# RaptorMai/online-continual-learning

Measured on NVIDIA H100. Metric: replay-step images/sec (ASER+SCR, ResNet18, CIFAR100), higher is better.
Workload: dtype f32

## Files before the change

include/b200ocl.h:

```cpp
#ifndef B200OCL_H_
#define B200OCL_H_

#include <stddef.h>
#include <stdint.h>

#ifdef __cplusplus
extern "C" {
#endif

#define B200OCL_OK 0
#define B200OCL_EINVAL 1
#define B200OCL_EUNSUPPORTED 2
#define B200OCL_EWORKSPACE 3
#define B200OCL_ECUDA 4

#define B200OCL_KNN_MAX_CAND 1024
#define B200OCL_KNN_MAX_CAND_LARGE 262144

const char* b200ocl_last_error(void);
int b200ocl_version(void);
uint64_t b200ocl_launch_count(void);
void b200ocl_profile_begin(void);
int b200ocl_profile_end(void);
int b200ocl_profile_get(int k, char* name, int name_len, double* ms, int* launches, double* work);
// ... 57 lines not shown
#define B200OCL_NET_MAX_DIM 4096

typedef struct {
  int in_h, in_w;
  int nf;
  int num_classes;
  int head;
  int feat_dim;
} b200ocl_net_desc;

typedef struct {
  float* params;
  float* grads;
  float* packed;
  float* bn_stats;
  int64_t* bn_tracked;
} b200ocl_net_state;

typedef struct {
  size_t n_params, n_packed, n_bn_stats;
  int n_bn, n_tensors, dim_in, out_dim;
} b200ocl_net_info;
int b200ocl_net_query(const b200ocl_net_desc* desc, b200ocl_net_info* info);
int b200ocl_net_tensor(const b200ocl_net_desc* desc, int i, size_t* offset, size_t* numel, int* has_grad);

int b200ocl_net_pack(const b200ocl_net_desc* desc, const b200ocl_net_state* st, void* stream);


size_t b200ocl_net_eval_workspace_bytes(const b200ocl_net_desc* desc, int N);
int b200ocl_net_features_eval(const b200ocl_net_desc* desc, const b200ocl_net_state* st, const float* x, int N,
                              float* feat, void* workspace, size_t workspace_bytes, void* stream);

size_t b200ocl_net_train_workspace_bytes(const b200ocl_net_desc* desc, int N);

typedef struct {
  size_t bytes;
  size_t z, a, mean, invstd;
  size_t feat, hid, proj;
  size_t wg_part, wg_layer;
  int cin, cout, ks, stride, hout, wout;
  int bn_fused, bn_grid;
  int wgrad_kernel, wgrad_splits;
  int sms;
} b200ocl_net_ws_layout;
int b200ocl_net_train_ws_layout(const b200ocl_net_desc* desc, int N, int layer, b200ocl_net_ws_layout* out);

typedef struct {
  int kernel;
  int nt, bn, pt, kwarps;
  int grid_x, grid_y;
  int th, tw, ti;
  size_t stat_bytes, stat_region;
  int sms;
} b200ocl_conv_geom;
int b200ocl_net_conv_geom(const b200ocl_net_desc* desc, int N, int layer, int pass, int sms, b200ocl_conv_geom* out);

int b200ocl_net_forward_train(const b200ocl_net_desc* desc, const b200ocl_net_state* st, const float* x, int N,
                              float* out, void* workspace, size_t workspace_bytes, void* stream);

int b200ocl_net_forward_evalgrad(const b200ocl_net_desc* desc, const b200ocl_net_state* st, const float* x, int N,
                                 float* out, void* workspace, size_t workspace_bytes, void* stream);

int b200ocl_net_forward_train_deferred(const b200ocl_net_desc* desc, const b200ocl_net_state* st, const float* x, int N,
                                       float* out, void* workspace, size_t workspace_bytes, void* stream);
int b200ocl_net_apply_running_stats(const b200ocl_net_desc* desc, const b200ocl_net_state* st, int N, void* workspace,
                                    size_t workspace_bytes, void* stream);

int b200ocl_net_backward(const b200ocl_net_desc* desc, const b200ocl_net_state* st, const float* x, const float* dout,
                         int N, void* workspace, size_t workspace_bytes, int accumulate, void* stream);

int b200ocl_net_sgd_step(const b200ocl_net_desc* desc, const b200ocl_net_state* st, float lr, float weight_decay,
                         const b200ocl_net_state* dst, void* stream);

size_t b200ocl_net_sgd_step_clipped_workspace_bytes(const b200ocl_net_desc* desc);
int b200ocl_net_sgd_step_clipped(const b200ocl_net_desc* desc, const b200ocl_net_state* st, float lr,
                                 float weight_decay, float max_norm, float* norm_out, void* workspace,
                                 size_t workspace_bytes, void* stream);

typedef struct {
  float* running;
  float* tmp;
  float* normalized;
  float* prev;
} b200ocl_ewc_state;

#define B200OCL_EWC_PENALTY 1
#define B200OCL_EWC_EMA 2

size_t b200ocl_net_sgd_step_ewc_workspace_bytes(const b200ocl_net_desc* desc);
int b200ocl_net_sgd_step_ewc(const b200ocl_net_desc* desc, const b200ocl_net_state* st, const b200ocl_ewc_state* ewc,
                             float lr, float weight_decay, float up, int flags, float ema_keep, float ema_add,
                             float* penalty_out, void* workspace, size_t workspace_bytes, void* stream);

typedef struct {
  float step_size, bc2_sqrt, bc2_sqrt_inv, eps, beta1_c, beta2, beta2_c, weight_decay, grad_scale;
} b200ocl_adam_scalars;

#define B200OCL_ADAM_FOREACH 1
#define B200OCL_ADAM_GRAD_SCALE 2

int b200ocl_adam_step(float* p, float* g, float* m, float* v, size_t n, const b200ocl_adam_scalars* s, int flags,
                      void* stream);

typedef struct {
  float* exp_avg;
  float* exp_avg_sq;
// ... 53 lines not shown
```

online-continual-learning_b200/csrc/conv.cu:

```cuda
#include "conv.cuh"

namespace b200ocl {
namespace {

constexpr int CONV_THREADS = 128;

__device__ __forceinline__ double warp_sum_d(double v) {
#pragma unroll
  for (int o = 16; o > 0; o >>= 1) v += __shfl_xor_sync(FULL_MASK, v, o);
  return v;
}

__device__ __forceinline__ void decode_pixel(const ConvArgs& a, int m, int& n, int& ho, int& wo) {
  if (a.parity_order) {
    const int hh = a.Hout >> 1, wh = a.Wout >> 1;
    const int mq = a.N * hh * wh;
    const int cls = m / mq;
    int idx = m - cls * mq;
    n = idx / (hh * wh);
    idx -= n * hh * wh;
    const int y = idx / wh;
    ho = 2 * y + (cls >> 1);
    wo = 2 * (idx - y * wh) + (cls & 1);
  } else {
// ... 634 lines not shown
  return B200OCL_OK;
}

int launch_stem(const ConvArgs& a, const ConvPlan& pl, cudaStream_t stream) {
  B200OCL_PROF(a.mode == CONV_EVAL ? "conv_eval" : "conv_train", 2.0 * a.M * 20.0 * 27.0, stream);
  stem_kernel<<<pl.grid_x, CONV_THREADS, 0, stream>>>(a);
  B200OCL_LAUNCHED();
  return B200OCL_OK;
}

ConvPlan none(const char* why) {
  ConvPlan pl{};
  pl.kernel = CONV_K_NONE;
  pl.why = why;
  return pl;
}

ConvPlan tiled(const ConvArgs& a, int kernel, int bn, int pt, int bm) {
  ConvPlan pl{};
  pl.kernel = kernel;
  pl.bn = bn;
  pl.pt = pt;
  pl.grid_x = (a.M + bm - 1) / bm;
  pl.grid_y = a.CN / bn;
  return pl;
}

}

ConvPlan conv_plan(const ConvArgs& a, int sms) {
  if (a.CK == 3) {
    if (a.CN != 20 || a.ks != 3 || a.stride != 1 || a.Hin != a.Hout || a.Win != a.Wout || a.M <= 0 || a.transposed)
      return none("only the 3->20 3x3 stride-1 stem is supported");
    return tiled(a, CONV_K_STEM, 20, 1, CONV_THREADS);
  }
  if (a.CK % 20 != 0 || a.CN % 20 != 0 || a.M <= 0) return none("channel counts must be multiples of 20");
  ConvPlan pl{};
  bool tcp = false, tc = false;
  if (a.force_path == 3) {
    if (!conv_tcp_eligible(a)) return none("launch not covered by the halo-patch tensor-core kernel (3x3 stride 1, no train mode)");
    tcp = true;
  } else if (a.force_path == 2) {
    if (!(a.w_tc && a.ks == 3 && a.stride == 1 && !a.transposed)) return none("shape not covered by conv_tc");
    tc = true;
  } else if (a.force_path == 0) {
    tcp = conv_tcp_eligible(a);
    tc = !tcp && conv_tc_eligible(a, sms);
  }
  if (tcp) {
    pl.kernel = CONV_K_TCP;
    pl.nt = a.tp_bn <= 20 ? 32 : 48;
    pl.grid_x = conv_tcp_grid_x(a, sms);
    pl.grid_y = a.CN / a.tp_bn;
    return pl;
  }
  if (tc) {
    pl.kernel = CONV_K_TC;
    pl.nt = a.tc_bn <= 20 ? 32 : (a.tc_bn <= 40 ? 48 : 80);
    pl.grid_x = (a.M + 127) / 128;
    pl.grid_y = a.CN / a.tc_bn;
    return pl;
  }
  if (!a.transposed && a.ks * a.ks * 20 * 80 * sizeof(float) <= 64 * 1024) {
    const long want3 = 5L * sms / 2;
    const int pbn[3] = {80, 40, 20};
    const int ppt[3] = {4, 2, 1};
    for (int pi = 0; pi < 3; ++pi)
      for (int bi = 0; bi < 3; ++bi) {
        if (a.CN % pbn[bi]) continue;
        const PatchTile t = patch_tile(a, pbn[bi], ppt[pi]);
        const long need = (ppt[pi] == 4) ? 3L * sms / 2 : want3;
        if (t.ctas < need || t.smem > (ppt[pi] == 4 ? 100 : 72) * 1024) continue;
        pl.kernel = CONV_K_PATCH;
        pl.bn = pbn[bi];
        pl.pt = ppt[pi];
        pl.grid_y = a.CN / pl.bn;
        pl.grid_x = (int)(t.ctas / pl.grid_y);
        pl.th = t.th; pl.tw = t.tw; pl.ti = t.ti;
        pl.smem = t.smem;
        return pl;
      }
  }
  const long want = 4L * sms;
  const int bns[3] = {80, 40, 20};
  auto ctas_reg = [&](int bn, int pt) {
    const int bm = (80 / bn) * 32 * pt;
    return (long)((a.M + bm - 1) / bm) * (a.CN / bn);
  };
  for (int bi = 0; bi < 3; ++bi)
    if (a.CN % bns[bi] == 0 && ctas_reg(bns[bi], 2) >= want) return tiled(a, CONV_K_TILED, bns[bi], 2, (80 / bns[bi]) * 64);
  if (a.ks * a.ks * (a.CK / 20) >= 4) {
    int pt = 1, kwarps = 4;
    const long ctas2 = (long)((a.M + 63) / 64) * (a.CN / 20);
    const long ctas1 = (long)((a.M + 31) / 32) * (a.CN / 20);
    if (ctas2 >= want) pt = 2;
    else if (ctas1 < 2L * sms && a.ks * a.ks * (a.CK / 20) >= 16) kwarps = 8;
    pl = tiled(a, CONV_K_KSPLIT, 20, pt, 32 * pt);
    pl.kwarps = kwarps;
    return pl;
  }
  return tiled(a, CONV_K_TILED, 20, 1, 128);
}

int launch_conv(const ConvArgs& a, int sms, cudaStream_t stream) {
  const ConvPlan pl = conv_plan(a, sms);
  switch (pl.kernel) {
// ... 33 lines not shown
```

online-continual-learning_b200/csrc/conv.cuh:

```cuda
#pragma once
#include "common.cuh"

namespace b200ocl {

enum ConvMode {
  CONV_RAW = 0,
  CONV_EVAL = 1,
  CONV_TRAIN = 2,
  CONV_ACCUM = 3
};

struct ConvArgs {
  const float* in;
  const float* w;
  float* out;
  int N, Hin, Win, CK, Hout, Wout, CN;
  int ks, stride, pad;
  int transposed;
  const float* w_tc;
  int tc_kb, tc_bn;
  const float* w_tp;
  int tp_bn, tp_slices;
  int tp_ps, tp_bs, tp_tiles;
  int force_path;
// ... 4 lines not shown
  int mode;
  const float* gamma;
  const float* beta;
  const float* rmean;
  const float* rvar;
  const float* residual;
  int relu;
  float eps;
  double* stat_part;
  unsigned int* counter;
  float* save_mean;
  float* save_invstd;
  float* run_mean;
  float* run_var;
  float momentum;
};

__device__ __forceinline__ float bn_running_update(float run, float s, float m) {
  return __fmaf_rn(1.f - m, run, __fmul_rn(m, s));
}

__device__ __forceinline__ void bn_finalize(const ConvArgs& a, int c, double S, double Q) {
  const double cnt = (double)a.M;
  const double mean = S / cnt;
  double var = Q / cnt - mean * mean;
  if (var < 0.0) var = 0.0;
  a.save_mean[c] = (float)mean;
  a.save_invstd[c] = (float)(1.0 / sqrt(var + (double)a.eps));
  const double unbiased = (a.M > 1) ? var * cnt / (cnt - 1.0) : var;
  a.run_mean[c] = bn_running_update(a.run_mean[c], (float)mean, a.momentum);
  a.run_var[c] = bn_running_update(a.run_var[c], (float)unbiased, a.momentum);
}

constexpr int TP_LD_MAX = 13;
inline bool tcp_strip_fits(int W) { return 128 + 2 * (W + 2) + 2 <= 16 * TP_LD_MAX; }

enum ConvKernel {
  CONV_K_NONE = -1,
  CONV_K_STEM = 0,
  CONV_K_TCP = 1,
  CONV_K_TC = 2,
  CONV_K_PATCH = 3,
  CONV_K_TILED = 4,
  CONV_K_KSPLIT = 5
};
struct ConvPlan {
  int kernel;
  int nt;
  int bn, pt;
  int kwarps;
  int grid_x, grid_y;
  int th, tw, ti;
  size_t smem;
  const char* why;
};
ConvPlan conv_plan(const ConvArgs& a, int sms);
inline size_t conv_stat_bytes(const ConvPlan& pl, int CN) { return (size_t)pl.grid_x * CN * 2 * sizeof(double); }
int launch_conv(const ConvArgs& a, int sms, cudaStream_t stream);
bool conv_tc_eligible(const ConvArgs& a, int sms);
int launch_conv_tc(const ConvArgs& a, const ConvPlan& pl, cudaStream_t stream);
bool conv_tcp_eligible(const ConvArgs& a);
int conv_tcp_grid_x(const ConvArgs& a, int sms);
int launch_conv_tcp(const ConvArgs& a, const ConvPlan& pl, cudaStream_t stream);

}
```

online-continual-learning_b200/csrc/conv_tcp.cu:

```cuda
#include "conv.cuh"
#include "umma.cuh"

namespace b200ocl {
namespace {

constexpr int TP_THREADS = 32 * 13;
constexpr int TP_LOADER_WARP = 9;
constexpr int TP_PS_MAX = 3;
constexpr int TP_BS_MAX = 6;
constexpr int TP_CONSUMER_WARPS = 8;

using umma::mbar_expect_tx;
using umma::bulk_g2s;

struct TileGeom {
  int wp, pp;
  int tiles_m;
  int prow;
  int pbytes;
};
__host__ __device__ inline TileGeom tile_geom(int N, int H, int W) {
  TileGeom g;
  g.wp = W + 1;
  g.pp = (H + 1) * (W + 1);
  const long last = (long)(N - 1) * g.pp + (long)(H - 1) * g.wp + (W - 1);
  g.tiles_m = (int)(last / 128) + 1;
  g.prow = 128 + 2 * g.wp + 2;
  g.pbytes = (g.prow * 128 + 1023) / 1024 * 1024;
  return g;
}

template <int NT, int KS>
__device__ __forceinline__ void issue_tap(float (&d)[NT / 2], uint64_t dAh, uint64_t dAl, uint64_t dBh, uint64_t dBl) {
  umma::fence();
#pragma unroll
  for (int k = 0; k < KS; ++k) {
    const uint64_t adv = (uint64_t)(k * 2);
    umma::mma_tf32_ss<NT>(d, dAh + adv, dBh + adv, k > 0 ? 1u : 0u);
    umma::mma_tf32_ss<NT>(d, dAh + adv, dBl + adv, 1u);
    umma::mma_tf32_ss<NT>(d, dAl + adv, dBh + adv, 1u);
  }
  umma::commit();
  umma::wait<0>();
  umma::fence_regs(d);
}

template <int NT>
__global__ void __launch_bounds__(TP_THREADS, 1) conv_tcp_kernel(ConvArgs a) {
  constexpr int B_BLOCK = 2 * NT * 32;
  constexpr int R = NT / 2;
  extern __shared__ __align__(1024) unsigned char smem_raw[];
  unsigned char* patch0 = smem_raw;
  __shared__ __align__(8) uint64_t pfull[TP_PS_MAX], pempty[TP_PS_MAX], bfull[9], bempty[TP_BS_MAX];
  __shared__ int s_fail;
  __shared__ float s_coef[3 * 80];

  const int tid = threadIdx.x, warp = tid >> 5;
  const int bn = a.tp_bn;
  const int n0 = blockIdx.y * bn;
  const int slices = a.tp_slices;
  const TileGeom G = tile_geom(a.N, a.Hin, a.Win);
  const int PS = a.tp_ps, BS = a.tp_bs;
  float* sB = reinterpret_cast<float*>(smem_raw + (size_t)PS * 2 * G.pbytes);
  const bool resident = (slices == 1 && NT == 32);
  const int b_slots = resident ? 9 : BS;
  float* s_acc = sB + (size_t)b_slots * B_BLOCK;

  if (tid == 0) {
    for (int i = 0; i < TP_PS_MAX; ++i) {
      umma::mbar_init(&pfull[i], 128);
      umma::mbar_init(&pempty[i], TP_CONSUMER_WARPS);
    }
    for (int i = 0; i < 9; ++i) umma::mbar_init(&bfull[i], 1);
    for (int i = 0; i < TP_BS_MAX; ++i) umma::mbar_init(&bempty[i], TP_CONSUMER_WARPS);
    umma::fence_mbar_init();
    s_fail = 0;
  }
  __syncthreads();
  const float* wimg = a.w_tp + (size_t)blockIdx.y * slices * 9 * B_BLOCK;

  if (warp >= TP_LOADER_WARP) {
    const int lt = tid - 32 * TP_LOADER_WARP;
    int pc = 0;
    for (int tile = blockIdx.x; tile < a.tp_tiles; tile += gridDim.x) {
      for (int sl = 0; sl < slices; ++sl, ++pc) {
        const int ch_valid = min(32, a.CK - sl * 32);
        const int nch = 2 * ((ch_valid + 7) / 8);
        const int ch = lt & 7, r0 = lt >> 3;
        const int nrow = G.prow;
        const bool ch_live = ch < nch, ch_real = ch * 4 < ch_valid;
        float4 v[TP_LD_MAX];
        int img, yp, xp;
        {
          const int sp = tile * 128 + r0;
          img = sp / G.pp;
          const int rem = sp - img * G.pp;
          yp = rem / G.wp;
          xp = rem - yp * G.wp;
        }
        const int hp = a.Hin + 1;
#pragma unroll
        for (int i = 0; i < TP_LD_MAX; ++i) {
          v[i] = make_float4(0.f, 0.f, 0.f, 0.f);
          const int ri = r0 + 16 * i;
          if (ch_real && ri < nrow) {
            const int y = yp - 1, x = xp - 1;
            if (img < a.N && (unsigned)y < (unsigned)a.Hin && (unsigned)x < (unsigned)a.Win)
              v[i] = __ldg(reinterpret_cast<const float4*>(a.in + ((size_t)(img * a.Hin + y) * a.Win + x) * a.CK + sl * 32) + ch);
          }
          xp += 16;
          while (xp >= G.wp) {
            xp -= G.wp;
            if (++yp == hp) {
              yp = 0;
              ++img;
            }
          }
        }
        const int ps = pc % PS;
        if (!umma::mbar_wait(&pempty[ps], (uint32_t)(((pc / PS) & 1) ^ 1))) s_fail = 1;
        float* ph = reinterpret_cast<float*>(patch0 + (size_t)ps * 2 * G.pbytes);
        float* pl = ph + G.pbytes / 4;
        if (ch_live) {
#pragma unroll
          for (int i = 0; i < TP_LD_MAX; ++i) {
            const int ri = r0 + 16 * i;
            if (ri < nrow) {
              float4 h, l;
              umma::split_tf32(v[i].x, h.x, l.x); umma::split_tf32(v[i].y, h.y, l.y);
              umma::split_tf32(v[i].z, h.z, l.z); umma::split_tf32(v[i].w, h.w, l.w);
              const int off = umma::sw128_offset_f32(ri, ch);
              *reinterpret_cast<float4*>(ph + off) = h;
              *reinterpret_cast<float4*>(pl + off) = l;
            }
          }
        }
        umma::fence_proxy_async_smem();
        umma::mbar_arrive(&pfull[ps]);
      }
    }
  } else if (warp == TP_LOADER_WARP - 1) {
    const uint32_t bytes = (uint32_t)(B_BLOCK * sizeof(float));
    if (resident) {
      if (umma::elect_one_sync()) {
        for (int b = 0; b < 9; ++b) {
          mbar_expect_tx(&bfull[b], bytes);
          bulk_g2s(sB + (size_t)b * B_BLOCK, wimg + (size_t)b * B_BLOCK, bytes, &bfull[b]);
        }
      }
    } else {
      int q = 0;
      for (int tile = blockIdx.x; tile < a.tp_tiles; tile += gridDim.x)
        for (int sl = 0; sl < slices; ++sl)
          for (int tap = 0; tap < 9; ++tap, ++q) {
            const int bs = q % BS;
            if (!umma::mbar_wait(&bempty[bs], (uint32_t)(((q / BS) & 1) ^ 1))) s_fail = 1;
            if (umma::elect_one_sync()) {
              mbar_expect_tx(&bfull[bs], bytes);
              bulk_g2s(sB + (size_t)bs * B_BLOCK, wimg + (size_t)(sl * 9 + tap) * B_BLOCK, bytes, &bfull[bs]);
            }
            __syncwarp();
          }
    }
  } else {
    const int g = warp >> 2, wt = tid & 127;
    const int et = tid;
    const bool epi = tid < 128;
    const bool lane0 = (tid & 31) == 0;
    auto esync = []() { asm volatile("bar.sync 1, 128;\n" ::); };
    auto csync = []() { asm volatile("bar.sync 2, 256;\n" ::); };
    const uint64_t dA0 = umma::make_smem_desc_sw128(umma::smem_u32(patch0) + (uint32_t)(g * 64 * 128));
    const uint64_t dB0 = umma::make_smem_desc_sw128(umma::smem_u32(sB));
    const uint32_t A_LO = (uint32_t)G.pbytes >> 4;
    const uint32_t A_STAGE = (uint32_t)(2 * G.pbytes) >> 4;
    constexpr uint32_t B_LO = (NT * 128) >> 4;
    constexpr uint32_t B_SLOT = (B_BLOCK * 4) >> 4;
    if (epi && a.mode == CONV_EVAL) {
      for (int c = et; c < bn; c += 128) {
        const float inv = 1.0f / sqrtf(a.rvar[n0 + c] + a.eps);
        s_coef[c] = a.rmean[n0 + c];
        s_coef[80 + c] = inv * a.gamma[n0 + c];
        s_coef[160 + c] = a.beta[n0 + c];
      }
      esync();
    }
    int pc = 0, q = 0;
    bool b_ready = false;
    for (int tile = blockIdx.x; tile < a.tp_tiles; tile += gridDim.x) {
      float accf[R];
#pragma unroll
      for (int i = 0; i < R; ++i) accf[i] = 0.f;
      for (int sl = 0; sl < slices; ++sl, ++pc) {
        const int ps = pc % PS;
        const int ksteps = (min(32, a.CK - sl * 32) + 7) / 8;
        if (!umma::mbar_wait(&pfull[ps], (uint32_t)((pc / PS) & 1))) s_fail = 1;
        const uint64_t dAs = dA0 + (uint64_t)(ps * A_STAGE);
#pragma unroll 1
        for (int tap = 0; tap < 9; ++tap, ++q) {
          const int kh = tap / 3, kw = tap - 3 * kh;
          const int b = resident ? tap : q % BS;
          if (!(resident && b_ready))
            if (!umma::mbar_wait(&bfull[b], resident ? 0u : (uint32_t)((q / BS) & 1))) s_fail = 1;
          const uint64_t dAh = dAs + (uint64_t)((kh * G.wp + kw) * 8);
          const uint64_t dAl = dAh + A_LO;
          const uint64_t dBh = dB0 + (uint64_t)(b * B_SLOT);
          const uint64_t dBl = dBh + B_LO;
          float tmp[R];
          switch (ksteps) {
            case 1: issue_tap<NT, 1>(tmp, dAh, dAl, dBh, dBl); break;
            case 2: issue_tap<NT, 2>(tmp, dAh, dAl, dBh, dBl); break;
            case 3: issue_tap<NT, 3>(tmp, dAh, dAl, dBh, dBl); break;
            default: issue_tap<NT, 4>(tmp, dAh, dAl, dBh, dBl); break;
          }
#pragma unroll
          for (int i = 0; i < R; ++i) accf[i] += tmp[i];
          if (!resident && lane0) umma::mbar_arrive(&bempty[b]);
        }
        b_ready = true;
        if (lane0) umma::mbar_arrive(&pempty[ps]);
      }
      csync();
#pragma unroll
      for (int i = 0; i < R; ++i) s_acc[(64 * g + umma::frag_row(wt, i)) * (NT + 1) + umma::frag_col(wt, i)] = accf[i];
      csync();
      if (!epi) continue;
      const int sp = tile * 128 + et;
      const int img = sp / G.pp, rem = sp - img * G.pp;
      const int y = rem / G.wp, x = rem - y * G.wp;
      const bool valid = img < a.N && y < a.Hin && x < a.Win;
      const size_t m = ((size_t)img * a.Hin + y) * a.Win + x;
      float acc[NT], pre[NT];
#pragma unroll
      for (int c = 0; c < NT; ++c) {
        acc[c] = 0.f;
        pre[c] = 0.f;
      }
      {
        const float* src = nullptr;
        if (valid && a.mode == CONV_EVAL && a.residual) src = a.residual + m * a.CN + n0;
        if (valid && a.mode == CONV_ACCUM) src = a.out + m * a.CN + n0;
        if (src) {
#pragma unroll
          for (int c0 = 0; c0 < NT; c0 += 4) {
            if (c0 >= bn) break;
            const float4 v = *reinterpret_cast<const float4*>(src + c0);
            pre[c0] = v.x; pre[c0 + 1] = v.y; pre[c0 + 2] = v.z; pre[c0 + 3] = v.w;
          }
        }
      }
#pragma unroll
      for (int c = 0; c < NT; ++c) acc[c] = s_acc[et * (NT + 1) + c];
      if (a.mode == CONV_EVAL) {
        if (valid) {
          float* o = a.out + m * a.CN + n0;
#pragma unroll
          for (int c0 = 0; c0 < NT; c0 += 4) {
            if (c0 >= bn) break;
            float rr[4];
#pragma unroll
            for (int j = 0; j < 4; ++j) {
              rr[j] = (acc[c0 + j] - s_coef[c0 + j]) * s_coef[80 + c0 + j] + s_coef[160 + c0 + j];
              rr[j] += pre[c0 + j];
              if (a.relu) rr[j] = fmaxf(rr[j], 0.f);
            }
            *reinterpret_cast<float4*>(o + c0) = make_float4(rr[0], rr[1], rr[2], rr[3]);
          }
        }
      } else if (valid) {
        float* o = a.out + m * a.CN + n0;
#pragma unroll
        for (int c0 = 0; c0 < NT; c0 += 4) {
          if (c0 >= bn) break;
          *reinterpret_cast<float4*>(o + c0) = make_float4(acc[c0] + pre[c0], acc[c0 + 1] + pre[c0 + 1],
                                                           acc[c0 + 2] + pre[c0 + 2], acc[c0 + 3] + pre[c0 + 3]);
        }
      }
    }
  }
  __syncthreads();
  if (s_fail && tid == 0) a.out[(size_t)n0] = __int_as_float(0x7fc00000);
}

template <int NT>
size_t tcp_smem_bytes(const TileGeom& G, int slices, int ps, int bs) {
  const int b_slots = (slices == 1 && NT == 32) ? 9 : bs;
  return (size_t)ps * 2 * G.pbytes + (size_t)b_slots * 2 * NT * 32 * sizeof(float) +
         (size_t)128 * (NT + 1) * sizeof(float) + 1024;
}

template <int NT>
int launch_tcp(ConvArgs a, const ConvPlan& pl, cudaStream_t stream) {
  const TileGeom G = tile_geom(a.N, a.Hin, a.Win);
  const size_t limit = 227 * 1024 - 4096
                       - (size_t)128 * (a.tp_bn + 1) * sizeof(float);
  a.tp_ps = 3; a.tp_bs = 6;
  if (tcp_smem_bytes<NT>(G, a.tp_slices, a.tp_ps, a.tp_bs) > limit) a.tp_bs = 4;
  if (tcp_smem_bytes<NT>(G, a.tp_slices, a.tp_ps, a.tp_bs) > limit) { a.tp_ps = 2; a.tp_bs = 6; }
  const size_t smem = tcp_smem_bytes<NT>(G, a.tp_slices, a.tp_ps, a.tp_bs);
  B200OCL_CUDA(raise_smem_limit<conv_tcp_kernel<NT>>(smem));
  a.tp_tiles = G.tiles_m;
  B200OCL_PROF("conv_tcp",
               2.0 * a.M * (double)a.CN * a.CK * 9.0, stream);
  conv_tcp_kernel<NT><<<dim3(pl.grid_x, pl.grid_y), TP_THREADS, smem, stream>>>(a);
  B200OCL_LAUNCHED();
  return B200OCL_OK;
}

}

int conv_tcp_grid_x(const ConvArgs& a, int sms) {
  const TileGeom G = tile_geom(a.N, a.Hin, a.Win);
  int gx = sms / (a.CN / a.tp_bn);
  if (gx < 1) gx = 1;
  if (gx > G.tiles_m) gx = G.tiles_m;
  const int rounds = (G.tiles_m + gx - 1) / gx;
  return (G.tiles_m + rounds - 1) / rounds;
}

bool conv_tcp_eligible(const ConvArgs& a) {
  if (a.mode == CONV_TRAIN || !a.w_tp || a.transposed || a.CK % 4 != 0) return false;
  if (a.ks != 3 || a.pad != 1 || a.stride != 1 || a.Hout != a.Hin || a.Wout != a.Win) return false;
  if (!tcp_strip_fits(a.Win)) return false;
  if ((long)a.N * (a.Hin + 2) * (a.Win + 2) > 2000000000L) return false;
  if (a.tp_bn <= 0 || a.tp_bn > 40 || a.CN % a.tp_bn != 0) return false;
  return true;
}

int launch_conv_tcp(const ConvArgs& a, const ConvPlan& pl, cudaStream_t stream) {
  if (pl.nt == 32) return launch_tcp<32>(a, pl, stream);
  return launch_tcp<48>(a, pl, stream);
}

}
```

online-continual-learning_b200/csrc/net_fwd.cu:

```cuda
#include <float.h>
#include <math.h>

#include "net_ws.cuh"
#include "umma.cuh"

namespace b200ocl {
namespace {

struct PackTable {
  int n;
  struct {
    unsigned int w_off, pkf_off, pkd_off;
    int cin, cout, taps;
  } e[NET_MAX_CONV];
};

__global__ void __launch_bounds__(256) pack_kernel(PackTable t, const float* __restrict__ params,
                                                   float* __restrict__ packed) {
  const auto& L = t.e[blockIdx.y];
  const int total = L.cout * L.cin * L.taps;
  for (int e = blockIdx.x * blockDim.x + threadIdx.x; e < total; e += gridDim.x * blockDim.x) {
    const int co = e / (L.cin * L.taps);
    const int rem = e - co * (L.cin * L.taps);
    const int ci = rem / L.taps, tap = rem - ci * L.taps;
// ... 1033 lines not shown
  c.hin = H; c.win = W;
  c.hout = b200ocl::conv_out(H, ks, stride, c.pad);
  c.wout = b200ocl::conv_out(W, ks, stride, c.pad);
  c.w_off = 0;
  pk = 0;
  b200ocl::conv_pack_layout(c, pk);
}

static b200ocl::ConvArgs selftest_args(const b200ocl::ConvL& c, int N, const float* x, const float* packed, float* out,
                                       int dgrad, int path, int mode) {
  using namespace b200ocl;
  ConvArgs a = conv_layer_args(c, N, x, packed, out, dgrad);
  a.mode = mode >= 3 ? CONV_EVAL : mode == 2 ? CONV_TRAIN : (mode == 1 ? CONV_ACCUM : CONV_RAW);
  a.force_path = path;
  return a;
}

static size_t selftest_stat_bytes(const b200ocl::ConvL& c, int N, int sms) {
  using namespace b200ocl;
  size_t stat = 0;
  for (int path = 0; path <= 2; ++path) {
    const ConvPlan pl = conv_plan(selftest_args(c, N, nullptr, nullptr, nullptr, 0, path, 2), sms);
    if (pl.kernel != CONV_K_NONE && conv_stat_bytes(pl, c.cout) > stat) stat = conv_stat_bytes(pl, c.cout);
  }
  return stat;
}

static size_t selftest_workspace_bytes(int N, int cin, int cout, int H, int W, int ks, int stride, int sms) {
  b200ocl::ConvL c;
  size_t pk = 0;
  selftest_layer(c, cin, cout, H, W, ks, stride, pk);
  const size_t stat = selftest_stat_bytes(c, N, sms);
  return b200ocl::align_up(pk * sizeof(float), 256) + b200ocl::align_up(stat, 256) + 256  + 256;
}

size_t b200ocl_conv_selftest_workspace_bytes(int N, int cin, int cout, int H, int W, int ks, int stride) {
  return selftest_workspace_bytes(N, cin, cout, H, W, ks, stride, b200ocl::sm_count());
}

static void report_geom(const b200ocl::ConvPlan& pl, size_t stat_bytes, size_t stat_region, int sms,
                        b200ocl_conv_geom* out) {
  *out = b200ocl_conv_geom{};
  out->kernel = pl.kernel;
  out->nt = pl.nt;
  out->bn = pl.bn;
  out->pt = pl.pt;
  out->kwarps = pl.kwarps;
  out->grid_x = pl.grid_x;
  out->grid_y = pl.grid_y;
  out->th = pl.th; out->tw = pl.tw; out->ti = pl.ti;
  out->stat_bytes = stat_bytes;
  out->stat_region = stat_region;
  out->sms = sms;
}

int b200ocl_conv_selftest_geom(int N, int H, int W, int cin, int cout, int ks, int stride, int dgrad, int path, int mode,
                               int sms, b200ocl_conv_geom* out) {
  using namespace b200ocl;
  B200OCL_CHECK_ARG(out, "null pointer");
  B200OCL_CHECK_ARG(N > 0 && H > 0 && W > 0 && cin % 20 == 0 && cout % 20 == 0 && cin > 0 && cout > 0, "bad shape");
  B200OCL_CHECK_ARG((ks == 3 || ks == 1) && (stride == 1 || stride == 2) && mode >= 0 && mode <= 4 && sms >= 0,
                    "3x3 or 1x1, stride 1 or 2, mode 0..4, sms >= 0");
  if (sms == 0) sms = sm_count();
  ConvL c;
  size_t pk = 0;
  selftest_layer(c, cin, cout, H, W, ks, stride, pk);
  const ConvPlan pl = conv_plan(selftest_args(c, N, nullptr, nullptr, nullptr, dgrad, path, mode), sms);
  const bool train = mode == 2 && pl.kernel != CONV_K_NONE;
  report_geom(pl, train ? conv_stat_bytes(pl, cout) : 0, selftest_stat_bytes(c, N, sms), sms, out);
  return B200OCL_OK;
}

int b200ocl_conv_selftest(const float* x, const float* w_oihw, float* out, int N, int H, int W, int cin, int cout,
                          int ks, int stride, int dgrad, int path, int mode, float* stats_out, void* workspace,
                          size_t workspace_bytes, void* stream_) {
  using namespace b200ocl;
  cudaStream_t stream = static_cast<cudaStream_t>(stream_);
  B200OCL_CHECK_ARG(x && w_oihw && out && workspace, "null pointer");
  B200OCL_CHECK_ARG(N > 0 && H > 0 && W > 0 && cin % 20 == 0 && cout % 20 == 0 && cin > 0 && cout > 0, "bad shape");
  B200OCL_CHECK_ARG(mode >= 0 && mode <= 4 && (mode != 2 || (stats_out && !dgrad)), "mode 2 (train) needs stats_out, forward only");
  B200OCL_CHECK_ARG(mode < 3 || (stats_out && !dgrad && (mode == 3 || cin == cout)),
                    "modes 3 / 4 (eval) need stats_out, forward only; mode 4 needs cin == cout");
  B200OCL_CHECK_ARG((ks == 3 || ks == 1) && (stride == 1 || stride == 2) && (!dgrad || (ks == 3 && stride == 1)),
                    "3x3 or 1x1, stride 1 or 2; data gradient for 3x3 stride 1 only");
  B200OCL_CHECK_ARG(workspace_bytes >= b200ocl_conv_selftest_workspace_bytes(N, cin, cout, H, W, ks, stride), "workspace too small");
  NetPlan p;
  memset(&p, 0, sizeof(p));
  p.n_conv = 1;
  size_t pk = 0;
  selftest_layer(p.conv[0], cin, cout, H, W, ks, stride, pk);
  p.n_packed = pk;
  unsigned char* base = static_cast<unsigned char*>(workspace);
  float* packed = reinterpret_cast<float*>(base);
  double* stat_part = reinterpret_cast<double*>(base + align_up(pk * sizeof(float), 256));
  const int sms = sm_count();
  const size_t stat = selftest_stat_bytes(p.conv[0], N, sms);
  unsigned int* counters = reinterpret_cast<unsigned int*>(reinterpret_cast<unsigned char*>(stat_part) + align_up(stat, 256));
  int rc = launch_pack(p, w_oihw, packed, stream);
  if (rc) return rc;
  ConvArgs a = selftest_args(p.conv[0], N, x, packed, out, dgrad, path, mode);
  a.eps = NET_BN_EPS;
  a.momentum = NET_BN_MOMENTUM;
  if (mode == 2) {
    B200OCL_CUDA(cudaMemsetAsync(counters, 0, 64, stream));
    B200OCL_CUDA(cudaMemsetAsync(stats_out, 0, (size_t)4 * cout * sizeof(float), stream));
    a.stat_part = stat_part;
// ... 475 lines not shown
```

online-continual-learning_b200/csrc/umma.cuh:

```cuda
#pragma once
#include <stdint.h>

namespace b200ocl {
namespace umma {

__device__ __forceinline__ uint32_t smem_u32(const void* p) {
  return static_cast<uint32_t>(__cvta_generic_to_shared(p));
}

__device__ __forceinline__ int sw128_offset_f32(int row, int chunk16) {
  return (row >> 3) * 256 + (row & 7) * 32 + ((chunk16 ^ (row & 7)) << 2);
}

__device__ __forceinline__ int frag_row(int t, int i) { return ((t >> 5) << 4) + ((t & 31) >> 2) + ((i & 2) << 2); }
__device__ __forceinline__ int frag_col(int t, int i) { return ((i >> 2) << 3) + ((t & 3) << 1) + (i & 1); }

__device__ __forceinline__ uint64_t make_smem_desc_sw128(uint32_t smem_addr) {
  uint64_t d = 0;
  d |= (uint64_t)((smem_addr >> 4) & 0x3FFF);
  d |= (uint64_t)1 << 16;
  d |= (uint64_t)((1024 >> 4) & 0x3FFF) << 32;
  d |= (uint64_t)1 << 62;
  return d;
}

__device__ __forceinline__ void fence() { asm volatile("wgmma.fence.sync.aligned;\n" ::: "memory"); }
__device__ __forceinline__ void commit() { asm volatile("wgmma.commit_group.sync.aligned;\n" ::: "memory"); }
template <int N>
__device__ __forceinline__ void wait() { asm volatile("wgmma.wait_group.sync.aligned %0;\n" ::"n"(N) : "memory"); }
template <int R>
__device__ __forceinline__ void fence_regs(float (&d)[R]) {
#pragma unroll
  for (int i = 0; i < R; ++i) asm volatile("" : "+f"(d[i])::"memory");
}
__device__ __forceinline__ void fence_proxy_async_smem() { asm volatile("fence.proxy.async.shared::cta;\n" ::); }

__device__ __forceinline__ void mbar_init(uint64_t* bar, uint32_t count) {
  asm volatile("mbarrier.init.shared::cta.b64 [%0], %1;\n" ::"r"(smem_u32(bar)), "r"(count));
}
__device__ __forceinline__ void fence_mbar_init() { asm volatile("fence.mbarrier_init.release.cluster;\n" ::); }
__device__ __forceinline__ bool mbar_wait(uint64_t* bar, uint32_t parity, uint32_t max_spins = (1u << 24)) {
  const uint32_t addr = smem_u32(bar);
#pragma unroll 1
  for (uint32_t i = 0; i < max_spins; ++i) {
    uint32_t done;
    asm volatile(
        "{\n\t.reg .pred p;\n\t"
        "mbarrier.try_wait.parity.shared::cta.b64 p, [%1], %2;\n\t"
        "selp.u32 %0, 1, 0, p;\n\t}\n"
        : "=r"(done)
        : "r"(addr), "r"(parity)
        : "memory");
    if (done) return true;
  }
  return false;
}
__device__ __forceinline__ void mbar_arrive(uint64_t* bar) {
  asm volatile("mbarrier.arrive.shared::cta.b64 _, [%0];\n" ::"r"(smem_u32(bar)) : "memory");
}

__device__ __forceinline__ void mbar_expect_tx(uint64_t* bar, uint32_t bytes) {
  asm volatile("mbarrier.arrive.expect_tx.shared::cta.b64 _, [%0], %1;\n" ::"r"(smem_u32(bar)), "r"(bytes)
               : "memory");
}
__device__ __forceinline__ void bulk_g2s(void* smem_dst, const void* gmem_src, uint32_t bytes, uint64_t* bar) {
  asm volatile(
      "cp.async.bulk.shared::cluster.global.mbarrier::complete_tx::bytes [%0], [%1], %2, [%3];\n" ::"r"(
          smem_u32(smem_dst)),
      "l"(gmem_src), "r"(bytes), "r"(smem_u32(bar))
      : "memory");
}

__device__ __forceinline__ bool elect_one_sync() {
  uint32_t pred;
  asm volatile(
      "{\n\t.reg .pred P;\n\t"
      "elect.sync _|P, 0xffffffff;\n\t"
      "selp.u32 %0, 1, 0, P;\n\t}\n"
      : "=r"(pred));
  return pred != 0;
}

template <int N>
__device__ __forceinline__ void mma_tf32_ss(float (&d)[N / 2], uint64_t desc_a, uint64_t desc_b, uint32_t accumulate);
template <int N>
__device__ __forceinline__ void mma_tf32_rs(float (&d)[N / 2], const uint32_t (&a)[4], uint64_t desc_b, uint32_t accumulate);

// ... 63 lines not shown
```

online-continual-learning_b200/engine.py:

```python
import ctypes
from ctypes import c_int, c_int64, c_size_t, c_void_p
from types import SimpleNamespace

import torch

from . import _native, ops
from .ops import _stream, _workspace, _need_cuda

HEAD_CODES = {None: 0, 'classifier': 0, 'linear': 1, 'mlp': 2, 'None': 3}


class NetDesc(ctypes.Structure):
    _fields_ = [('in_h', c_int), ('in_w', c_int), ('nf', c_int), ('num_classes', c_int), ('head', c_int),
                ('feat_dim', c_int)]


class NetState(ctypes.Structure):
    _fields_ = [('params', c_void_p), ('grads', c_void_p), ('packed', c_void_p), ('bn_stats', c_void_p),
                ('bn_tracked', c_void_p)]


class EwcState(ctypes.Structure):
    _fields_ = [('running', c_void_p), ('tmp', c_void_p), ('normalized', c_void_p), ('prev', c_void_p)]


class AdamState(ctypes.Structure):
    _fields_ = [('exp_avg', c_void_p), ('exp_avg_sq', c_void_p)]


class NetInfo(ctypes.Structure):
    _fields_ = [('n_params', c_size_t), ('n_packed', c_size_t), ('n_bn_stats', c_size_t), ('n_bn', c_int),
                ('n_tensors', c_int), ('dim_in', c_int), ('out_dim', c_int)]


class NetWsLayout(ctypes.Structure):
    _fields_ = [('bytes', c_size_t), ('z', c_size_t), ('a', c_size_t), ('mean', c_size_t), ('invstd', c_size_t),
                ('feat', c_size_t), ('hid', c_size_t), ('proj', c_size_t), ('wg_part', c_size_t), ('wg_layer', c_size_t),
                ('cin', c_int), ('cout', c_int), ('ks', c_int), ('stride', c_int), ('hout', c_int), ('wout', c_int),
                ('bn_fused', c_int), ('bn_grid', c_int), ('wgrad_kernel', c_int), ('wgrad_splits', c_int), ('sms', c_int)]


class ConvGeom(ctypes.Structure):
    _fields_ = [('kernel', c_int), ('nt', c_int), ('bn', c_int), ('pt', c_int), ('kwarps', c_int), ('grid_x', c_int),
                ('grid_y', c_int), ('th', c_int), ('tw', c_int), ('ti', c_int), ('stat_bytes', c_size_t),
                ('stat_region', c_size_t), ('sms', c_int)]

    KERNELS = ('stem', 'tcp', 'tc', 'patch', 'tiled', 'ksplit')

    @property
    def name(self):
        return self.KERNELS[self.kernel] if self.kernel >= 0 else 'none'

    @property
    def template(self):
        return {'stem': ('stem',), 'tcp': ('tcp', self.nt), 'tc': ('tc', self.nt), 'patch': ('patch', self.bn, self.pt),
                'tiled': ('tiled', self.bn, self.pt), 'ksplit': ('ksplit', self.pt, self.kwarps),
                'none': ('none',)}[self.name]


CONV_PASSES = {'train': 0, 'eval': 1, 'dgrad': 2}


def _lib():
    return _native.lib()


def train_ws_layout(desc, n, layer):
    out = NetWsLayout()
    _native.check(_lib().b200ocl_net_train_ws_layout(ctypes.byref(desc), int(n), int(layer), ctypes.byref(out)),
                  'b200ocl_net_train_ws_layout')
    return out


def conv_geom(desc, n, layer, pass_, sms=0):
    out = ConvGeom()
    _native.check(_lib().b200ocl_net_conv_geom(ctypes.byref(desc), int(n), int(layer), CONV_PASSES[pass_], int(sms),
                                               ctypes.byref(out)), 'b200ocl_net_conv_geom')
    return out


def conv_selftest_geom(n, h, w, cin, cout, ks, stride, dgrad, path, mode, sms=0):
    out = ConvGeom()
    _native.check(_lib().b200ocl_conv_selftest_geom(int(n), int(h), int(w), int(cin), int(cout), int(ks), int(stride),
                                                    int(dgrad), int(path), int(mode), int(sms), ctypes.byref(out)),
                  'b200ocl_conv_selftest_geom')
    return out


def describe(in_hw, num_classes, head=None, feat_dim=128, nf=20):
    desc = NetDesc(int(in_hw), int(in_hw), int(nf), int(num_classes), HEAD_CODES[head], int(feat_dim))
    info = NetInfo()
    lib = _lib()
    _native.check(lib.b200ocl_net_query(ctypes.byref(desc), ctypes.byref(info)), 'b200ocl_net_query')
    table = []
    off, num, hg = c_size_t(), c_size_t(), c_int()
    for i in range(info.n_tensors):
        _native.check(lib.b200ocl_net_tensor(ctypes.byref(desc), i, ctypes.byref(off), ctypes.byref(num),
                                             ctypes.byref(hg)), 'b200ocl_net_tensor')
# ... 411 lines not shown
```

Before: 2099.

## Warp-specialize halo-patch conv kernel with separate epilogue warpgroup and async MMA overlap

The halo-patch tensor-core conv kernel is restructured into warp-specialized roles. A dedicated 128-thread epilogue warpgroup drains a double-buffered accumulator staging area through mbarriers, so the MMA warps no longer stall on the BN/residual epilogue. The MMA warps now keep one wgmma group in flight with two alternating fragment buffers instead of waiting after every tap. Register budgets are redistributed via setmaxnreg, the loader warps shrink from 128 to 96 threads, and the extra shared memory for two accumulator buffers may reduce pipeline depth. The chosen pipeline depth is also exposed in the geometry query.

```diff
diff --git a/include/b200ocl.h b/include/b200ocl.h
--- a/include/b200ocl.h
+++ b/include/b200ocl.h
@@ -133,6 +133,7 @@
   int th, tw, ti;
   size_t stat_bytes, stat_region;
   int sms;
+  int tp_ps, tp_bs;
 } b200ocl_conv_geom;
 int b200ocl_net_conv_geom(const b200ocl_net_desc* desc, int N, int layer, int pass, int sms, b200ocl_conv_geom* out);
 
diff --git a/online-continual-learning_b200/csrc/conv.cu b/online-continual-learning_b200/csrc/conv.cu
--- a/online-continual-learning_b200/csrc/conv.cu
+++ b/online-continual-learning_b200/csrc/conv.cu
@@ -710,6 +710,7 @@
     pl.nt = a.tp_bn <= 20 ? 32 : 48;
     pl.grid_x = conv_tcp_grid_x(a, sms);
     pl.grid_y = a.CN / a.tp_bn;
+    conv_tcp_pipeline(a, pl.nt, &pl.tp_ps, &pl.tp_bs);
     return pl;
   }
   if (tc) {
diff --git a/online-continual-learning_b200/csrc/conv.cuh b/online-continual-learning_b200/csrc/conv.cuh
--- a/online-continual-learning_b200/csrc/conv.cuh
+++ b/online-continual-learning_b200/csrc/conv.cuh
@@ -80,6 +80,7 @@
   int grid_x, grid_y;
   int th, tw, ti;
   size_t smem;
+  int tp_ps, tp_bs;
   const char* why;
 };
 ConvPlan conv_plan(const ConvArgs& a, int sms);
@@ -89,6 +90,7 @@
 int launch_conv_tc(const ConvArgs& a, const ConvPlan& pl, cudaStream_t stream);
 bool conv_tcp_eligible(const ConvArgs& a);
 int conv_tcp_grid_x(const ConvArgs& a, int sms);
+void conv_tcp_pipeline(const ConvArgs& a, int nt, int* ps, int* bs);
 int launch_conv_tcp(const ConvArgs& a, const ConvPlan& pl, cudaStream_t stream);
 
 }
diff --git a/online-continual-learning_b200/csrc/conv_tcp.cu b/online-continual-learning_b200/csrc/conv_tcp.cu
--- a/online-continual-learning_b200/csrc/conv_tcp.cu
+++ b/online-continual-learning_b200/csrc/conv_tcp.cu
@@ -4,11 +4,18 @@
 namespace b200ocl {
 namespace {
 
-constexpr int TP_THREADS = 32 * 13;
-constexpr int TP_LOADER_WARP = 9;
+constexpr int TP_THREADS = 32 * 16;
+constexpr int TP_EPI_WARP = 8;
+constexpr int TP_WLOAD_WARP = 12;
+constexpr int TP_LOADER_WARP = 13;
+constexpr int TP_LOADERS = 96;
+constexpr int TP_LD = (16 * TP_LD_MAX + 11) / 12;
 constexpr int TP_PS_MAX = 3;
 constexpr int TP_BS_MAX = 6;
 constexpr int TP_CONSUMER_WARPS = 8;
+constexpr int TP_REG_LOAD = 128, TP_REG_MMA = 144, TP_REG_EPI = 96;
+static_assert(TP_REG_LOAD == 128, "the loader warpgroup runs no setmaxnreg");
+static_assert(128 * TP_REG_LOAD + 256 * TP_REG_MMA + 128 * TP_REG_EPI <= 65536, "register file");
 
 using umma::mbar_expect_tx;
 using umma::bulk_g2s;
@@ -41,8 +48,6 @@
     umma::mma_tf32_ss<NT>(d, dAl + adv, dBh + adv, 1u);
   }
   umma::commit();
-  umma::wait<0>();
-  umma::fence_regs(d);
 }
 
 template <int NT>
@@ -52,6 +57,7 @@
   extern __shared__ __align__(1024) unsigned char smem_raw[];
   unsigned char* patch0 = smem_raw;
   __shared__ __align__(8) uint64_t pfull[TP_PS_MAX], pempty[TP_PS_MAX], bfull[9], bempty[TP_BS_MAX];
+  __shared__ __align__(8) uint64_t afull[2], aempty[2];
   __shared__ int s_fail;
   __shared__ float s_coef[3 * 80];
 
@@ -64,15 +70,20 @@
   float* sB = reinterpret_cast<float*>(smem_raw + (size_t)PS * 2 * G.pbytes);
   const bool resident = (slices == 1 && NT == 32);
   const int b_slots = resident ? 9 : BS;
+  constexpr int ACC_TILE = 128 * (NT + 1);
   float* s_acc = sB + (size_t)b_slots * B_BLOCK;
 
   if (tid == 0) {
     for (int i = 0; i < TP_PS_MAX; ++i) {
-      umma::mbar_init(&pfull[i], 128);
+      umma::mbar_init(&pfull[i], TP_LOADERS);
       umma::mbar_init(&pempty[i], TP_CONSUMER_WARPS);
     }
     for (int i = 0; i < 9; ++i) umma::mbar_init(&bfull[i], 1);
     for (int i = 0; i < TP_BS_MAX; ++i) umma::mbar_init(&bempty[i], TP_CONSUMER_WARPS);
+    for (int i = 0; i < 2; ++i) {
+      umma::mbar_init(&afull[i], 256);
+      umma::mbar_init(&aempty[i], 128);
+    }
     umma::fence_mbar_init();
     s_fail = 0;
   }
@@ -89,7 +100,7 @@
         const int ch = lt & 7, r0 = lt >> 3;
         const int nrow = G.prow;
         const bool ch_live = ch < nch, ch_real = ch * 4 < ch_valid;
-        float4 v[TP_LD_MAX];
+        float4 v[TP_LD];
         int img, yp, xp;
         {
           const int sp = tile * 128 + r0;
@@ -100,15 +111,15 @@
         }
         const int hp = a.Hin + 1;
 #pragma unroll
-        for (int i = 0; i < TP_LD_MAX; ++i) {
+        for (int i = 0; i < TP_LD; ++i) {
           v[i] = make_float4(0.f, 0.f, 0.f, 0.f);
-          const int ri = r0 + 16 * i;
+          const int ri = r0 + 12 * i;
           if (ch_real && ri < nrow) {
             const int y = yp - 1, x = xp - 1;
             if (img < a.N && (unsigned)y < (unsigned)a.Hin && (unsigned)x < (unsigned)a.Win)
               v[i] = __ldg(reinterpret_cast<const float4*>(a.in + ((size_t)(img * a.Hin + y) * a.Win + x) * a.CK + sl * 32) + ch);
           }
-          xp += 16;
+          xp += 12;
           while (xp >= G.wp) {
             xp -= G.wp;
             if (++yp == hp) {
@@ -123,8 +134,8 @@
         float* pl = ph + G.pbytes / 4;
         if (ch_live) {
 #pragma unroll
-          for (int i = 0; i < TP_LD_MAX; ++i) {
-            const int ri = r0 + 16 * i;
+          for (int i = 0; i < TP_LD; ++i) {
+            const int ri = r0 + 12 * i;
             if (ri < nrow) {
               float4 h, l;
               umma::split_tf32(v[i].x, h.x, l.x); umma::split_tf32(v[i].y, h.y, l.y);
@@ -139,7 +150,7 @@
         umma::mbar_arrive(&pfull[ps]);
       }
     }
-  } else if (warp == TP_LOADER_WARP - 1) {
+  } else if (warp == TP_WLOAD_WARP) {
     const uint32_t bytes = (uint32_t)(B_BLOCK * sizeof(float));
     if (resident) {
       if (umma::elect_one_sync()) {
@@ -162,119 +173,156 @@
             __syncwarp();
           }
     }
+  } else if (warp >= TP_EPI_WARP) {
+    umma::reg_dealloc<TP_REG_EPI>();
+    const int et = tid - 32 * TP_EPI_WARP;
+    if (a.mode == CONV_EVAL) {
+      for (int c = et; c < bn; c += 128) {
+        const float inv = 1.0f / sqrtf(a.rvar[n0 + c] + a.eps);
+        s_coef[c] = a.rmean[n0 + c];
+        s_coef[80 + c] = inv * a.gamma[n0 + c];
+        s_coef[160 + c] = a.beta[n0 + c];
+      }
+      asm volatile("bar.sync 1, 128;\n" ::);
+    }
+    int k = 0;
+    for (int tile = blockIdx.x; tile < a.tp_tiles; tile += gridDim.x, ++k) {
+      const int buf = k & 1;
+      const int sp = tile * 128 + et;
+      const int img = sp / G.pp, rem = sp - img * G.pp;
+      const int y = rem / G.wp, x = rem - y * G.wp;
+      const bool valid = img < a.N && y < a.Hin && x < a.Win;
+      const size_t m = ((size_t)img * a.Hin + y) * a.Win + x;
+      const float* src = nullptr;
+      if (valid && a.mode == CONV_EVAL && a.residual) src = a.residual + m * a.CN + n0;
+      if (valid && a.mode == CONV_ACCUM) src = a.out + m * a.CN + n0;
+      float pre[NT];
+#pragma unroll
+      for (int c = 0; c < NT; ++c) pre[c] = 0.f;
+      if (src) {
+#pragma unroll
+        for (int c0 = 0; c0 < NT; c0 += 4) {
+          if (c0 >= bn) break;
+          const float4 v = *reinterpret_cast<const float4*>(src + c0);
+          pre[c0] = v.x; pre[c0 + 1] = v.y; pre[c0 + 2] = v.z; pre[c0 + 3] = v.w;
+        }
+      }
+      if (!umma::mbar_wait(&afull[buf], (uint32_t)((k >> 1) & 1))) s_fail = 1;
+      const float* row = s_acc + (size_t)buf * ACC_TILE + et * (NT + 1);
+      if (valid) {
+        float* o = a.out + m * a.CN + n0;
+#pragma unroll
+        for (int c0 = 0; c0 < NT; c0 += 4) {
+          if (c0 >= bn) break;
+          float rr[4];
+#pragma unroll
+          for (int j = 0; j < 4; ++j) {
+            const float acc = row[c0 + j];
+            if (a.mode == CONV_EVAL) {
+              rr[j] = (acc - s_coef[c0 + j]) * s_coef[80 + c0 + j] + s_coef[160 + c0 + j];
+              rr[j] += pre[c0 + j];
+              if (a.relu) rr[j] = fmaxf(rr[j], 0.f);
+            } else {
+              rr[j] = acc + pre[c0 + j];
+            }
+          }
+          *reinterpret_cast<float4*>(o + c0) = make_float4(rr[0], rr[1], rr[2], rr[3]);
+        }
+      }
+      umma::mbar_arrive(&aempty[buf]);
+    }
   } else {
+    umma::reg_alloc<TP_REG_MMA>();
     const int g = warp >> 2, wt = tid & 127;
-    const int et = tid;
-    const bool epi = tid < 128;
     const bool lane0 = (tid & 31) == 0;
-    auto esync = []() { asm volatile("bar.sync 1, 128;\n" ::); };
-    auto csync = []() { asm volatile("bar.sync 2, 256;\n" ::); };
     const uint64_t dA0 = umma::make_smem_desc_sw128(umma::smem_u32(patch0) + (uint32_t)(g * 64 * 128));
     const uint64_t dB0 = umma::make_smem_desc_sw128(umma::smem_u32(sB));
     const uint32_t A_LO = (uint32_t)G.pbytes >> 4;
     const uint32_t A_STAGE = (uint32_t)(2 * G.pbytes) >> 4;
     constexpr uint32_t B_LO = (NT * 128) >> 4;
     constexpr uint32_t B_SLOT = (B_BLOCK * 4) >> 4;
-    if (epi && a.mode == CONV_EVAL) {
-      for (int c = et; c < bn; c += 128) {
-        const float inv = 1.0f / sqrtf(a.rvar[n0 + c] + a.eps);
-        s_coef[c] = a.rmean[n0 + c];
-        s_coef[80 + c] = inv * a.gamma[n0 + c];
-        s_coef[160 + c] = a.beta[n0 + c];
-      }
-      esync();
-    }
-    int pc = 0, q = 0;
+    const int T = 9 * slices;
+    int ips = 0, ib = 0, rps = 0, rb = 0;
+    uint32_t ipph = 0, ibph = 0;
     bool b_ready = false;
-    for (int tile = blockIdx.x; tile < a.tp_tiles; tile += gridDim.x) {
+    int k = 0;
+    for (int tile = blockIdx.x; tile < a.tp_tiles; tile += gridDim.x, ++k) {
       float accf[R];
 #pragma unroll
       for (int i = 0; i < R; ++i) accf[i] = 0.f;
-      for (int sl = 0; sl < slices; ++sl, ++pc) {
-        const int ps = pc % PS;
-        const int ksteps = (min(32, a.CK - sl * 32) + 7) / 8;
-        if (!umma::mbar_wait(&pfull[ps], (uint32_t)((pc / PS) & 1))) s_fail = 1;
-        const uint64_t dAs = dA0 + (uint64_t)(ps * A_STAGE);
+      int is = 0, it = 0, rt = 0;
+      auto issue = [&](float (&d)[R]) {
+        if (it == 0)
+          if (!umma::mbar_wait(&pfull[ips], ipph)) s_fail = 1;
+        const int b = resident ? it : ib;
+        if (!(resident && b_ready))
+          if (!umma::mbar_wait(&bfull[b], resident ? 0u : ibph)) s_fail = 1;
+        const int kh = it / 3, kw = it - 3 * kh;
+        const uint64_t dAh = dA0 + (uint64_t)(ips * A_STAGE) + (uint64_t)((kh * G.wp + kw) * 8);
+        const uint64_t dAl = dAh + A_LO;
+        const uint64_t dBh = dB0 + (uint64_t)(b * B_SLOT);
+        const uint64_t dBl = dBh + B_LO;
+        switch ((min(32, a.CK - is * 32) + 7) / 8) {
+          case 1: issue_tap<NT, 1>(d, dAh, dAl, dBh, dBl); break;
+          case 2: issue_tap<NT, 2>(d, dAh, dAl, dBh, dBl); break;
+          case 3: issue_tap<NT, 3>(d, dAh, dAl, dBh, dBl); break;
+          default: issue_tap<NT, 4>(d, dAh, dAl, dBh, dBl); break;
+        }
+        if (!resident && ++ib == BS) {
+          ib = 0;
+          ibph ^= 1u;
+        }
+        if (++it == 9) {
+          it = 0;
+          ++is;
+          b_ready = true;
+          if (++ips == PS) {
+            ips = 0;
+            ipph ^= 1u;
+          }
+        }
+      };
+      auto retire = [&](float (&d)[R]) {
+        umma::fence_regs(d);
+#pragma unroll
+        for (int i = 0; i < R; ++i) accf[i] += d[i];
+        if (!resident) {
+          if (lane0) umma::mbar_arrive(&bempty[rb]);
+          if (++rb == BS) rb = 0;
+        }
+        if (rt == 8) {
+          if (lane0) umma::mbar_arrive(&pempty[rps]);
+          if (++rps == PS) rps = 0;
+        }
+        if (++rt == 9) rt = 0;
+      };
+      float fa[R], fb[R];
+      issue(fa);
 #pragma unroll 1
-        for (int tap = 0; tap < 9; ++tap, ++q) {
-          const int kh = tap / 3, kw = tap - 3 * kh;
-          const int b = resident ? tap : q % BS;
-          if (!(resident && b_ready))
-            if (!umma::mbar_wait(&bfull[b], resident ? 0u : (uint32_t)((q / BS) & 1))) s_fail = 1;
-          const uint64_t dAh = dAs + (uint64_t)((kh * G.wp + kw) * 8);
-          const uint64_t dAl = dAh + A_LO;
-          const uint64_t dBh = dB0 + (uint64_t)(b * B_SLOT);
-          const uint64_t dBl = dBh + B_LO;
-          float tmp[R];
-          switch (ksteps) {
-            case 1: issue_tap<NT, 1>(tmp, dAh, dAl, dBh, dBl); break;
-            case 2: issue_tap<NT, 2>(tmp, dAh, dAl, dBh, dBl); break;
-            case 3: issue_tap<NT, 3>(tmp, dAh, dAl, dBh, dBl); break;
-            default: issue_tap<NT, 4>(tmp, dAh, dAl, dBh, dBl); break;
-          }
-#pragma unroll
-          for (int i = 0; i < R; ++i) accf[i] += tmp[i];
-          if (!resident && lane0) umma::mbar_arrive(&bempty[b]);
-        }
-        b_ready = true;
-        if (lane0) umma::mbar_arrive(&pempty[ps]);
-      }
-      csync();
-#pragma unroll
-      for (int i = 0; i < R; ++i) s_acc[(64 * g + umma::frag_row(wt, i)) * (NT + 1) + umma::frag_col(wt, i)] = accf[i];
-      csync();
-      if (!epi) continue;
-      const int sp = tile * 128 + et;
-      const int img = sp / G.pp, rem = sp - img * G.pp;
-      const int y = rem / G.wp, x = rem - y * G.wp;
-      const bool valid = img < a.N && y < a.Hin && x < a.Win;
-      const size_t m = ((size_t)img * a.Hin + y) * a.Win + x;
-      float acc[NT], pre[NT];
-#pragma unroll
-      for (int c = 0; c < NT; ++c) {
-        acc[c] = 0.f;
-        pre[c] = 0.f;
-      }
-      {
-        const float* src = nullptr;
-        if (valid && a.mode == CONV_EVAL && a.residual) src = a.residual + m * a.CN + n0;
-        if (valid && a.mode == CONV_ACCUM) src = a.out + m * a.CN + n0;
-        if (src) {
-#pragma unroll
-          for (int c0 = 0; c0 < NT; c0 += 4) {
-            if (c0 >= bn) break;
-            const float4 v = *reinterpret_cast<const float4*>(src + c0);
-            pre[c0] = v.x; pre[c0 + 1] = v.y; pre[c0 + 2] = v.z; pre[c0 + 3] = v.w;
-          }
-        }
-      }
-#pragma unroll
-      for (int c = 0; c < NT; ++c) acc[c] = s_acc[et * (NT + 1) + c];
-      if (a.mode == CONV_EVAL) {
-        if (valid) {
-          float* o = a.out + m * a.CN + n0;
-#pragma unroll
-          for (int c0 = 0; c0 < NT; c0 += 4) {
-            if (c0 >= bn) break;
-            float rr[4];
-#pragma unroll
-            for (int j = 0; j < 4; ++j) {
-              rr[j] = (acc[c0 + j] - s_coef[c0 + j]) * s_coef[80 + c0 + j] + s_coef[160 + c0 + j];
-              rr[j] += pre[c0 + j];
-              if (a.relu) rr[j] = fmaxf(rr[j], 0.f);
-            }
-            *reinterpret_cast<float4*>(o + c0) = make_float4(rr[0], rr[1], rr[2], rr[3]);
-          }
-        }
-      } else if (valid) {
-        float* o = a.out + m * a.CN + n0;
-#pragma unroll
-        for (int c0 = 0; c0 < NT; c0 += 4) {
-          if (c0 >= bn) break;
-          *reinterpret_cast<float4*>(o + c0) = make_float4(acc[c0] + pre[c0], acc[c0 + 1] + pre[c0 + 1],
-                                                           acc[c0 + 2] + pre[c0 + 2], acc[c0 + 3] + pre[c0 + 3]);
-        }
-      }
+      for (int j = 0;; j += 2) {
+        if (j + 1 >= T) {
+          umma::wait<0>();
+          retire(fa);
+          break;
+        }
+        issue(fb);
+        umma::wait<1>();
+        retire(fa);
+        if (j + 2 >= T) {
+          umma::wait<0>();
+          retire(fb);
+          break;
+        }
+        issue(fa);
+        umma::wait<1>();
+        retire(fb);
+      }
+      const int buf = k & 1;
+      if (!umma::mbar_wait(&aempty[buf], (uint32_t)(((k >> 1) & 1) ^ 1))) s_fail = 1;
+      float* acc_out = s_acc + (size_t)buf * ACC_TILE;
+#pragma unroll
+      for (int i = 0; i < R; ++i) acc_out[(64 * g + umma::frag_row(wt, i)) * (NT + 1) + umma::frag_col(wt, i)] = accf[i];
+      umma::mbar_arrive(&afull[buf]);
     }
   }
   __syncthreads();
@@ -285,17 +333,23 @@
 size_t tcp_smem_bytes(const TileGeom& G, int slices, int ps, int bs) {
   const int b_slots = (slices == 1 && NT == 32) ? 9 : bs;
   return (size_t)ps * 2 * G.pbytes + (size_t)b_slots * 2 * NT * 32 * sizeof(float) +
-         (size_t)128 * (NT + 1) * sizeof(float) + 1024;
+         (size_t)2 * 128 * (NT + 1) * sizeof(float) + 1024;
+}
+
+template <int NT>
+void fit_pipeline(const ConvArgs& a, int* ps, int* bs) {
+  const TileGeom G = tile_geom(a.N, a.Hin, a.Win);
+  const size_t limit = 227 * 1024 - 4096;
+  *ps = 3; *bs = 6;
+  if (tcp_smem_bytes<NT>(G, a.tp_slices, *ps, *bs) > limit) *bs = 4;
+  if (tcp_smem_bytes<NT>(G, a.tp_slices, *ps, *bs) > limit) { *ps = 2; *bs = 6; }
+  if (tcp_smem_bytes<NT>(G, a.tp_slices, *ps, *bs) > limit) *bs = 4;
 }
 
 template <int NT>
 int launch_tcp(ConvArgs a, const ConvPlan& pl, cudaStream_t stream) {
   const TileGeom G = tile_geom(a.N, a.Hin, a.Win);
-  const size_t limit = 227 * 1024 - 4096
-                       - (size_t)128 * (a.tp_bn + 1) * sizeof(float);
-  a.tp_ps = 3; a.tp_bs = 6;
-  if (tcp_smem_bytes<NT>(G, a.tp_slices, a.tp_ps, a.tp_bs) > limit) a.tp_bs = 4;
-  if (tcp_smem_bytes<NT>(G, a.tp_slices, a.tp_ps, a.tp_bs) > limit) { a.tp_ps = 2; a.tp_bs = 6; }
+  fit_pipeline<NT>(a, &a.tp_ps, &a.tp_bs);
   const size_t smem = tcp_smem_bytes<NT>(G, a.tp_slices, a.tp_ps, a.tp_bs);
   B200OCL_CUDA(raise_smem_limit<conv_tcp_kernel<NT>>(smem));
   a.tp_tiles = G.tiles_m;
@@ -308,6 +362,11 @@
 
 }
 
+void conv_tcp_pipeline(const ConvArgs& a, int nt, int* ps, int* bs) {
+  if (nt == 32) fit_pipeline<32>(a, ps, bs);
+  else fit_pipeline<48>(a, ps, bs);
+}
+
 int conv_tcp_grid_x(const ConvArgs& a, int sms) {
   const TileGeom G = tile_geom(a.N, a.Hin, a.Win);
   int gx = sms / (a.CN / a.tp_bn);
diff --git a/online-continual-learning_b200/csrc/net_fwd.cu b/online-continual-learning_b200/csrc/net_fwd.cu
--- a/online-continual-learning_b200/csrc/net_fwd.cu
+++ b/online-continual-learning_b200/csrc/net_fwd.cu
@@ -1109,6 +1109,8 @@
   out->stat_bytes = stat_bytes;
   out->stat_region = stat_region;
   out->sms = sms;
+  out->tp_ps = pl.tp_ps;
+  out->tp_bs = pl.tp_bs;
 }
 
 int b200ocl_conv_selftest_geom(int N, int H, int W, int cin, int cout, int ks, int stride, int dgrad, int path, int mode,
diff --git a/online-continual-learning_b200/csrc/umma.cuh b/online-continual-learning_b200/csrc/umma.cuh
--- a/online-continual-learning_b200/csrc/umma.cuh
+++ b/online-continual-learning_b200/csrc/umma.cuh
@@ -33,6 +33,10 @@
 #pragma unroll
   for (int i = 0; i < R; ++i) asm volatile("" : "+f"(d[i])::"memory");
 }
+template <int N>
+__device__ __forceinline__ void reg_dealloc() { asm volatile("setmaxnreg.dec.sync.aligned.u32 %0;\n" ::"n"(N)); }
+template <int N>
+__device__ __forceinline__ void reg_alloc() { asm volatile("setmaxnreg.inc.sync.aligned.u32 %0;\n" ::"n"(N)); }
 __device__ __forceinline__ void fence_proxy_async_smem() { asm volatile("fence.proxy.async.shared::cta;\n" ::); }
 
 __device__ __forceinline__ void mbar_init(uint64_t* bar, uint32_t count) {
diff --git a/online-continual-learning_b200/engine.py b/online-continual-learning_b200/engine.py
--- a/online-continual-learning_b200/engine.py
+++ b/online-continual-learning_b200/engine.py
@@ -43,7 +43,7 @@
 class ConvGeom(ctypes.Structure):
     _fields_ = [('kernel', c_int), ('nt', c_int), ('bn', c_int), ('pt', c_int), ('kwarps', c_int), ('grid_x', c_int),
                 ('grid_y', c_int), ('th', c_int), ('tw', c_int), ('ti', c_int), ('stat_bytes', c_size_t),
-                ('stat_region', c_size_t), ('sms', c_int)]
+                ('stat_region', c_size_t), ('sms', c_int), ('tp_ps', c_int), ('tp_bs', c_int)]
 
     KERNELS = ('stem', 'tcp', 'tc', 'patch', 'tiled', 'ksplit')
 
```

Result: faster. 2181 (median of 6 runs) (+3.9%).
